# jenkinsm13/julia-spira

Hardware: AMD Instinct MI355X
Metric: Msamples/sec at 1920x1080 spp=64 depth=8; fraction of HBM roofline (higher is better)
Workload: dtype f64

## Files before the change

### julia-spira_amd/csrc/spira_device.h

```cpp
#pragma once
#include <hip/hip_runtime.h>
#include <stdint.h>
#include <type_traits>
#include "spira_fastdiv.h"
#include "spira_sky.h"

namespace spira {

__device__ __forceinline__ float sqrt_rn(float x) { return __builtin_sqrtf(x); }
__device__ __forceinline__ double sqrt_rn(double x) { return __builtin_sqrt(x); }

constexpr int kBlock = 256;
#ifndef SPIRA_WAVES_F32
#define SPIRA_WAVES_F32 5
#endif
#ifndef SPIRA_WAVES_F64
#define SPIRA_WAVES_F64 4
#endif
#define SPIRA_WAVES_PER_SIMD(T) (sizeof(T) == 8 ? SPIRA_WAVES_F64 : SPIRA_WAVES_F32)
constexpr uint32_t kMaxTries = 64;

template <class T> struct Vec { T x, y, z; };

template <class T> __device__ __forceinline__ Vec<T> mk(T x, T y, T z) { Vec<T> r; r.x = x; r.y = y; r.z = z; return r; }
// ... 830 lines not shown
        n = mk<T>(sc.tri[3 * ti].w, sc.tri[3 * ti + 1].w, sc.tri[3 * ti + 2].w);
    } else {
        const Pack4<T> e1p = sc.bvh_tris[3 * (size_t)slot + 1], e2p = sc.bvh_tris[3 * (size_t)slot + 2];
        n = normalize(cross(mk<T>(e1p.x, e1p.y, e1p.z), mk<T>(e2p.x, e2p.y, e2p.z)));
    }
    const int mi = material_of<T, BVH, TRI>(sc, prim, slot);
    const Pack4<T> ma = sc.mat[2 * mi], mb = sc.mat[2 * mi + 1];
    Vec<T> diffuse = mk<T>(ma.x, ma.y, ma.z), emission = mk<T>(mb.x, mb.y, mb.z);
    T specular = ma.w, roughness = mb.w;
    if (EXT && (ext->flags & kExtSpectral)) {
        const T sd = ext_uplift<T>(*ext, diffuse), se = ext_uplift<T>(*ext, emission);
        diffuse = mk<T>(sd, sd, sd); emission = mk<T>(se, se, se);
    }
    const bool has_contrib = (emission.x != 0 || emission.y != 0 || emission.z != 0);
    contrib = mulv(beta, emission);
    pend.kind = kDead; pend.rough = 0; pend.v = mk<T>(0, 0, 0);
    if (scatter) {
        if (EXT && (ext->flags & kExtDielectric) && roughness < (T)0.0) {
            pend.v = n; pend.kind = kDielectric; pend.rough = -roughness;
            beta = mulv(beta, diffuse);
        } else if (specular > (T)0.0) {
            pend.v = d - n * ((T)2 * dot(d, n));
            pend.kind = roughness > (T)0.0 ? kSpecRough : kMirror;
            pend.rough = roughness;
            beta = mulv(beta * specular, diffuse);
        } else {
            pend.v = pos + n;
            pend.kind = kDiffuse;
            beta = mulv(beta * (T)0.5, diffuse);
        }
    }
    return has_contrib;
}

template <class T, bool BVH, bool EXT = false>
__device__ __forceinline__ bool shade_hit(const SceneLds<T> &sc, const Vec<T> pos, const Vec<T> d, int prim, uint32_t slot, Vec<T> &beta,
                                          bool scatter, Vec<T> &contrib, Pending<T> &pend, const ExtState<T> *ext = nullptr) {
    ExactDiv exact;
    return shade_hit<T, BVH, EXT>(sc, pos, d, prim, slot, beta, scatter, contrib, pend, ext, exact);
}

template <class T>
__device__ __forceinline__ void dielectric_resolve(Pending<T> &pend, const Vec<T> d, const RngKey &key) {
    const Vec<T> n = pend.v;
    const T ior = pend.rough;
    const T cosd = dot(d, n);
    const bool entering = cosd < (T)0.0;
    const Vec<T> nn = entering ? n : mk<T>(-n.x, -n.y, -n.z);
    const T eta = entering ? (T)1.0 / ior : ior;
    const T ci = entering ? -cosd : cosd;
    const T s2 = (eta * eta) * ((T)1.0 - ci * ci);
    T r0 = ((T)1.0 - ior) / ((T)1.0 + ior); r0 = r0 * r0;
    const T x = (T)1.0 - ci, x2 = x * x;
    const T refl = r0 + ((T)1.0 - r0) * ((x2 * x2) * x);
    T u, u1, u2;
    rng3<T>(key, 1, u, u1, u2);
    if (s2 > (T)1.0 || u < refl) pend.v = d - nn * ((T)2 * dot(d, nn));
    else pend.v = d * eta + nn * (eta * ci - sqrt_rn((T)1.0 - s2));
    pend.kind = kMirror;
}

template <class T, bool BVH, bool EXT = false>
__device__ __forceinline__ SegInfo segment_front(const SceneLds<T> &sc, Vec<T> &o, const Vec<T> d, Vec<T> &beta, bool scatter,
                                                 Vec<T> &contrib, T &t_out, Pending<T> &pend, const ExtState<T> *ext = nullptr) {
    SegInfo info;
    T t;
    uint32_t slot;
    int prim = closest_hit<T, BVH>(sc, o, d, (T)0.001, t, slot);
    info.prim = prim;
    t_out = prim >= 0 ? t : (T)0;
    if (prim < 0) {
        pend.kind = kDead; pend.rough = 0; pend.v = mk<T>(0, 0, 0);
        contrib = sky_term_x<T, EXT>(d, beta, ext);
        info.alive = false; info.has_contrib = true;
        return info;
    }
    const Vec<T> pos = o + d * t;
    info.has_contrib = shade_hit<T, BVH, EXT>(sc, pos, d, prim, slot, beta, scatter, contrib, pend, ext);
    info.alive = scatter;
    if (scatter) o = pos;
    return info;
}

template <class T, class P>
__device__ __forceinline__ Vec<T> segment_back(const Vec<T> pos, const Pending<T> &pend, const Vec<T> rnd, P &pol) {
    if (pend.kind == kDiffuse) return normalize((pend.v + rnd) - pos, pol);
    Vec<T> reflected = pend.v;
    if (pend.kind == kSpecRough) reflected = reflected + rnd * pend.rough;
    return normalize(reflected, pol);
}
template <class T>
__device__ __forceinline__ Vec<T> segment_back(const Vec<T> pos, const Pending<T> &pend, const Vec<T> rnd) {
    ExactDiv exact;
    return segment_back<T>(pos, pend, rnd, exact);
}

template <class T, bool BVH, bool EXT = false>
__device__ __forceinline__ SegInfo trace_segment(const SceneLds<T> &sc, const RenderConst<T> &rc, Vec<T> &o, Vec<T> &d,
                                                 Vec<T> &beta, uint32_t pixel, uint32_t sample, uint32_t bounce,
                                                 bool scatter, Vec<T> &contrib, T &t_out, const ExtState<T> *ext = nullptr) {
    Pending<T> pend;
    const Vec<T> d_in = d;
    SegInfo info = segment_front<T, BVH, EXT>(sc, o, d, beta, scatter, contrib, t_out, pend, ext);
    if (info.alive) {
        Vec<T> rnd = mk<T>(0, 0, 0);
        if (EXT && pend.kind == kDielectric) dielectric_resolve<T>(pend, d_in, rng_key(rc.sA, rc.sB, pixel, sample, bounce));
        if (pend.kind == kDiffuse || pend.kind == kSpecRough)
            rnd = random_in_unit_sphere<T>(rng_key(rc.sA, rc.sB, pixel, sample, bounce));
        d = segment_back<T>(o, pend, rnd);
    }
    return info;
}

template <class T, class P>
__device__ __forceinline__ void camera_ray(const RenderConst<T> &rc, uint32_t i, uint32_t j, uint32_t pixel, uint32_t sample,
                                           Vec<T> &o, Vec<T> &d, P &pol) {
    T xu, xv, unused;
    rng3<T>(rng_key(rc.sA, rc.sB, pixel, sample, 0), 0, xu, xv, unused);
    T u = ((T)(i - 1) + xu) / (T)(rc.width - 1);
    T v = ((T)(j - 1) + xv) / (T)(rc.height - 1);
    o = rc.cam_origin;
    d = normalize(((rc.cam_llc + rc.cam_hor * u) + rc.cam_ver * v) - o, pol);
}
template <class T>
__device__ __forceinline__ void camera_ray(const RenderConst<T> &rc, uint32_t i, uint32_t j, uint32_t pixel, uint32_t sample,
                                           Vec<T> &o, Vec<T> &d) {
    ExactDiv exact;
    camera_ray<T>(rc, i, j, pixel, sample, o, d, exact);
}
__device__ __forceinline__ float to_scalar(float x) { return __uint_as_float(__builtin_amdgcn_readfirstlane(__float_as_uint(x))); }
__device__ __forceinline__ double to_scalar(double x) {
    const uint32_t lo = __builtin_amdgcn_readfirstlane((uint32_t)__double2loint(x)), hi = __builtin_amdgcn_readfirstlane((uint32_t)__double2hiint(x));
    return __hiloint2double((int)hi, (int)lo);
}
template <class T> struct PixelDiv { Recip<T> w1, h1; };
template <class T> __device__ __forceinline__ PixelDiv<T> pixel_divisors(const RenderConst<T> &rc) {
    PixelDiv<T> p;
    p.w1 = recip_of((T)(rc.width - 1)); p.h1 = recip_of((T)(rc.height - 1));
    p.w1.d = to_scalar(p.w1.d); p.w1.r = to_scalar(p.w1.r); p.h1.d = to_scalar(p.h1.d); p.h1.r = to_scalar(p.h1.r);
    return p;
}
template <class T> __device__ __forceinline__ T pixel_quotient(T n, const Recip<T> &rc, ExactDiv &) { return n / rc.d; }
template <class T> __device__ __forceinline__ T pixel_quotient(T n, const Recip<T> &rc, SpecDiv &) { return quotient(n, rc); }
template <class T, class P>
__device__ __forceinline__ void camera_ray_lds(const RenderConst<T> &rc, const T *cam, const PixelDiv<T> &pd, uint32_t i, uint32_t j, uint32_t pixel, uint32_t sample,
                                               Vec<T> &o, Vec<T> &d, P &pol) {
    T xu, xv, unused;
    rng3<T>(rng_key(rc.sA, rc.sB, pixel, sample, 0), 0, xu, xv, unused);
    T u = pixel_quotient<T>((T)(i - 1) + xu, pd.w1, pol);
    T v = pixel_quotient<T>((T)(j - 1) + xv, pd.h1, pol);
    o = mk<T>(cam[0], cam[1], cam[2]);
    const Vec<T> llc = mk<T>(cam[3], cam[4], cam[5]), hor = mk<T>(cam[6], cam[7], cam[8]), ver = mk<T>(cam[9], cam[10], cam[11]);
    d = normalize(((llc + hor * u) + ver * v) - o, pol);
}

template <class T>
__device__ __forceinline__ void path_of(const RenderConst<T> &rc, uint32_t q, uint32_t pass, uint32_t &i, uint32_t &j,
                                        uint32_t &pixel, uint32_t &sample) {
    uint32_t slot = fastdiv(q, rc.fd_tile);
    uint32_t pl = q - slot * rc.tile_pixels;
    uint32_t lr = fastdiv(pl, rc.fd_width);
    uint32_t lx = pl - lr * rc.width;
    j = ref_row_j(rc, lr);
    i = lx + 1;
    pixel = (j - 1) * rc.width + lx;
    sample = rc.sample0 + pass * rc.slots + slot;
}

template <class T> struct RayQueue { Pack4<T> *A; Pack4<T> *B; Pack2<T> *C; };

struct Stats {
    unsigned long long segments, rays_enqueued, radiance_rmw, radiance_store, redone_waves, rays_parked;
// ... 271 lines not shown
    uint32_t pass;
    uint32_t n_first;
    uint32_t dense_pct;
    Pack4<T> *mesh_list;
    uint32_t mesh_min_batch;
    uint32_t refill_free;
    uint32_t mesh_mode;
    uint32_t *mesh_count;
    uint32_t resume_k, resume_nw;
    uint32_t *redo;
    uint32_t redo_only;
    Stats *stats;
    Pack4<T> *accum;
    FastDiv fd_keff;
    uint32_t k_eff;
    uint32_t accum_first;
    uint32_t l_private;
    uint32_t sky_runs;
};

#ifndef SPIRA_RESOLVE_RUN
#define SPIRA_RESOLVE_RUN 4
#endif
__device__ __forceinline__ uint32_t owned_pixel(uint32_t w, uint32_t nw, uint32_t l) {
    constexpr uint32_t kRun = SPIRA_RESOLVE_RUN;
    static_assert(64 % kRun == 0, "a run length divides the wave");
    return ((l / kRun) * nw + w) * kRun + l % kRun;
}

template <class T>
__device__ __forceinline__ void resolve_pixel(Pack4<T> *accum, const Pack3<T> *L, uint32_t tile_pixels, uint32_t k_eff, bool first_pass, uint32_t p) {
    Pack4<T> acc;
    if (first_pass) { acc.x = 0; acc.y = 0; acc.z = 0; acc.w = 0; } else acc = accum[p];
    uint32_t s = 0;
    for (; s + 8 <= k_eff; s += 8) {
        Pack3<T> l[8];
#pragma unroll
        for (int k = 0; k < 8; ++k) l[k] = L[(size_t)(s + k) * tile_pixels + p];
#pragma unroll
        for (int k = 0; k < 8; ++k) { acc.x = acc.x + l[k].x; acc.y = acc.y + l[k].y; acc.z = acc.z + l[k].z; }
    }
    for (; s < k_eff; ++s) {
        const Pack3<T> l = L[(size_t)s * tile_pixels + p];
        acc.x = acc.x + l.x; acc.y = acc.y + l.y; acc.z = acc.z + l.z;
    }
    accum[p] = acc;
}
template <class T>
__device__ __forceinline__ void resolve_pixel_run(Pack4<T> *accum, const Pack3<T> *Lp, uint32_t k_eff, bool first_pass, uint32_t p) {
    constexpr uint32_t kRun = SPIRA_RESOLVE_RUN;
    Pack4<T> acc;
    if (first_pass) { acc.x = 0; acc.y = 0; acc.z = 0; acc.w = 0; } else acc = accum[p];
    uint32_t s = 0;
    for (; s + 8 <= k_eff; s += 8) {
        Pack3<T> l[8];
#pragma unroll
        for (int k = 0; k < 8; ++k) l[k] = Lp[(s + k) * kRun];
#pragma unroll
        for (int k = 0; k < 8; ++k) { acc.x = acc.x + l[k].x; acc.y = acc.y + l[k].y; acc.z = acc.z + l[k].z; }
    }
    for (; s < k_eff; ++s) {
        const Pack3<T> l = Lp[s * kRun];
        acc.x = acc.x + l.x; acc.y = acc.y + l.y; acc.z = acc.z + l.z;
    }
    accum[p] = acc;
}

__device__ __forceinline__ float pack_qref(uint32_t q, uint32_t, float) { return __uint_as_float(q); }
__device__ __forceinline__ double pack_qref(uint32_t q, uint32_t ref, double) { return __longlong_as_double((long long)((unsigned long long)q | ((unsigned long long)ref << 32))); }
__device__ __forceinline__ uint32_t unpack_q(float w) { return __float_as_uint(w); }
__device__ __forceinline__ uint32_t unpack_q(double w) { return (uint32_t)(unsigned long long)__double_as_longlong(w); }
__device__ __forceinline__ uint32_t unpack_ref(double w) { return (uint32_t)((unsigned long long)__double_as_longlong(w) >> 32); }

#ifdef SPIRA_MESH_STATS
__device__ unsigned long long g_mesh_dbg[32];
#define MESH_STAT(...) __VA_ARGS__
#else
#define MESH_STAT(...)
#endif

#ifndef SPIRA_CARRY_KEY
#define SPIRA_CARRY_KEY 1
#endif
#ifndef SPIRA_WAVES_B_F32
#define SPIRA_WAVES_B_F32 4
#endif
#ifndef SPIRA_WAVES_B_F64
#define SPIRA_WAVES_B_F64 SPIRA_WAVES_F64
#endif
#ifndef SPIRA_WAVES_PATH_F32
#define SPIRA_WAVES_PATH_F32 6
#endif
template <class T, int R, bool BVH, bool EXT, bool SPEC, int MODE = 0, bool TRI = true>
__global__ __launch_bounds__(kBlock, MODE == 2 ? (sizeof(T) == 8 ? SPIRA_WAVES_B_F64 : SPIRA_WAVES_B_F32) : (sizeof(T) == 4 ? SPIRA_WAVES_PATH_F32 : SPIRA_WAVES_F64)) void k_path(const PathArgs<T> a) {
    extern __shared__ __attribute__((aligned(32))) unsigned char lds_raw[];
    constexpr uint32_t WPB = kBlock / 64, SUB = 64 * R;
    constexpr bool kRefArray = sizeof(T) == 4;
    constexpr bool kCarry = SPIRA_CARRY_KEY && !BVH && !EXT;
    constexpr uint32_t kStageShift = 25, kRefMask = (1u << kStageShift) - 1u;
    const uint32_t lane = threadIdx.x & 63, wave = threadIdx.x >> 6;
    const uint32_t NW = gridDim.x * WPB, wid = blockIdx.x * WPB + wave;
    const RenderConst<T> &rc = a.rc;
    using Pol = typename std::conditional<SPEC, SpecDiv, ExactDiv>::type;
    Pol pol;
    if (!SPEC && a.redo_only) {
        uint32_t any = 0;
        for (uint32_t w = 0; w < WPB; ++w) any |= a.redo[blockIdx.x * WPB + w];
        if (!any) return;
    }
    T *cam_lds = reinterpret_cast<T *>(lds_raw + scene_lds_bytes<T>(a.scene.n_spheres, a.scene.n_materials, a.scene.n_triangles) + WPB * SUB * sizeof(Pack4<T>));
    if (threadIdx.x < 12) {
        const Vec<T> *cv = threadIdx.x < 3 ? &rc.cam_origin : (threadIdx.x < 6 ? &rc.cam_llc : (threadIdx.x < 9 ? &rc.cam_hor : &rc.cam_ver));
        const uint32_t cc = threadIdx.x % 3;
        cam_lds[threadIdx.x] = cc == 0 ? cv->x : (cc == 1 ? cv->y : cv->z);
    }
    Pack4<T> *cam_sph = reinterpret_cast<Pack4<T> *>(reinterpret_cast<unsigned char *>(cam_lds) + 128);
    constexpr bool kCam = !EXT;
    if (kCam && MODE != 2 && a.cam_consts)
        for (uint32_t i = threadIdx.x; i < a.scene.n_spheres; i += blockDim.x) {
            const T *sp = a.scene.spheres5 + 5 * (size_t)i;
            const Vec<T> oc = rc.cam_origin - mk<T>(sp[0], sp[1], sp[2]);
            Pack4<T> k; k.x = oc.x; k.y = oc.y; k.z = oc.z; k.w = dot(oc, oc) - sp[3] * sp[3];
            cam_sph[i] = k;
        }
    const SceneLds<T> sc = stage_scene<T>(a.scene, lds_raw);
    const PixelDiv<T> pix_div = pixel_divisors<T>(rc);
    if (!SPEC && a.redo_only) {
        if (!a.redo[wid]) return;
        if (lane == 0) atomicAdd(&a.stats->redone_waves, 1ull);
    }
    Pack4<T> *s_rnd = reinterpret_cast<Pack4<T> *>(lds_raw + scene_lds_bytes<T>(a.scene.n_spheres, a.scene.n_materials, a.scene.n_triangles)) + wave * SUB;
    constexpr uint32_t mesh_mode = BVH ? (uint32_t)MODE : 0u;
    const uint32_t kseg = mesh_mode == 2u ? a.resume_k : 1u;
    if (mesh_mode == 2u && wid * kseg >= a.resume_nw) return;
    const uint32_t region = wid * kseg * a.cap;
    const unsigned long long lt_mask = (1ull << lane) - 1ull;
    const uint32_t ref_base = sc.n_spheres + sc.n_triangles;
    const bool mixed = mesh_mode != 0u || rc.max_depth <= 128u;
    const uint32_t dense_pct = mixed ? a.dense_pct : 0u;
    const bool defer = mesh_mode != 0u || (BVH && mixed && a.mesh_list != nullptr);
    Pack4<T> *mlist = a.mesh_list + 3 * (size_t)region;
    uint32_t n_rmw = 0, n_store = 0, n_seg = 0, n_enq = 0, n_park = 0;
    uint32_t n_wtrips = 0, n_ltrips = 0;
    uint32_t n_in = 0;
    const bool own = !BVH && !EXT && !TRI && sizeof(T) == 8 && a.accum != nullptr;
    const uint32_t n_own = own ? 64u * a.k_eff : 0u;
    const uint32_t n_sub_first = own ? (n_own + SUB - 1) / SUB : (a.n_first + SUB - 1) / SUB;
    const bool priv = kCarry && own && a.l_private != 0;
    const uint32_t l_base = priv ? wid * n_own : 0u;
    constexpr bool kOwnT = !BVH && !EXT && !TRI && sizeof(T) == 8;
    uint32_t sky_mask = 0;
    uint32_t *sky_word = reinterpret_cast<uint32_t *>(cam_lds + 12) + wave;
    static_assert(12 * sizeof(T) + WPB * sizeof(uint32_t) <= 128 || !kOwnT, "a word per wave behind the camera");
    if constexpr (kOwnT) {
        if (own && a.sky_runs) {
            constexpr uint32_t kRun = SPIRA_RESOLVE_RUN, kRuns = 64 / kRun, kRowSlots = 64 / kRun;
            static_assert(kRun == 4 && 2 * 64 * sizeof(Pack3<T>) <= SUB * sizeof(Pack4<T>), "the run mask below is written for runs of 4; a row of terms fits the work list");
            {
                const uint32_t px = owned_pixel(wid, NW, lane);
                bool sky = false;
                if (px < rc.tile_pixels) {
                    uint32_t pi, pj, pixel, sample;
                    path_of<T>(rc, px, a.pass, pi, pj, pixel, sample);
                    sky = sky_pixel(cam_lds, rc.width, rc.height, pi, pj, a.scene.spheres5, a.scene.n_spheres);
                }
                unsigned long long b = __ballot(sky);
                b &= b >> 1; b &= b >> 2;
                for (uint32_t g = 0; g < kRuns; ++g) sky_mask |= (uint32_t)((b >> (kRun * g)) & 1ull) << g;
            }
            Pack3<T> *s_sky = reinterpret_cast<Pack3<T> *>(s_rnd);
            for (uint32_t m = sky_mask; m; m &= m - 1u) {
                const uint32_t g = (uint32_t)__builtin_ctz(m);
                const uint32_t px = owned_pixel(wid, NW, g * kRun + lane % kRun);
                uint32_t pi, pj, pixel, sample0;
                path_of<T>(rc, px, a.pass, pi, pj, pixel, sample0);
                Pack3<T> acc;
                acc.x = 0; acc.y = 0; acc.z = 0;
                if (!a.accum_first && lane < kRun) { const Pack4<T> a0 = a.accum[px]; acc.x = a0.x; acc.y = a0.y; acc.z = a0.z; }
                for (uint32_t s0 = 0; s0 < a.k_eff; s0 += kRowSlots) {
                    const uint32_t slot = s0 + lane / kRun;
                    if (slot < a.k_eff) {
                        Vec<T> o_, d_;
                        camera_ray_lds<T>(rc, cam_lds, pix_div, pi, pj, pixel, sample0 + slot, o_, d_, pol);
                        const Vec<T> c = sky_term_x<T, EXT>(d_, mk<T>(1, 1, 1), nullptr);
                        Pack3<T> l; l.x = c.x; l.y = c.y; l.z = c.z;
                        s_sky[lane] = l;
                        ++n_seg; ++n_store;
                    }
                    wave_lds_sync();
                    if (lane < kRun) {
                        const uint32_t n = a.k_eff - s0 < kRowSlots ? a.k_eff - s0 : kRowSlots;
                        for (uint32_t k = 0; k < n; ++k) { const Pack3<T> l = s_sky[k * kRun + lane]; acc.x = acc.x + l.x; acc.y = acc.y + l.y; acc.z = acc.z + l.z; }
                    }
                    wave_lds_sync();
                }
                if (lane < kRun) a.L[priv ? l_base + g * a.k_eff * kRun + lane : px] = acc;
            }
        }
        if (own) { if (lane == 0) *sky_word = sky_mask; wave_lds_sync(); }
    }

    auto park = [&](uint32_t slot_i, const Vec<T> o_, const Vec<T> d_, const Vec<T> beta_, T closest_, uint32_t q_, int prim_, uint32_t stage_hit) {
        Pack4<T> A, B, C;
        A.x = o_.x; A.y = o_.y; A.z = o_.z; A.w = d_.x;
        B.x = d_.y; B.y = d_.z; B.z = beta_.x; B.w = beta_.y;
        C.x = beta_.z; C.y = closest_; C.z = Bits<T>::from_u32(q_); C.w = Bits<T>::from_u32((uint32_t)(prim_ + 1) | (stage_hit << kStageShift));
        mlist[3 * (size_t)slot_i] = A; mlist[3 * (size_t)slot_i + 1] = B; mlist[3 * (size_t)slot_i + 2] = C;
    };
    uint32_t mfill = 0;
    constexpr int kMaxSeg = 16;
    uint32_t pfx[kMaxSeg + 1];
    bool segmented = false;
    {
        uint32_t cnt = 0;
        if (mesh_mode == 2u && lane < kseg && wid * kseg + lane < a.resume_nw) cnt = a.mesh_count[wid * kseg + lane];
        pfx[0] = 0;
#pragma unroll
        for (int j = 0; j < kMaxSeg; ++j) pfx[j + 1] = pfx[j] + (uint32_t)__builtin_amdgcn_readlane((int)cnt, j);
        if (mesh_mode == 2u) { mfill = pfx[kMaxSeg]; segmented = true; }
    }
    const uint32_t first_sub = own ? 0u : (mesh_mode == 1u ? (wid % a.resume_k) * (NW / a.resume_k) + wid / a.resume_k : wid);
    const uint32_t sub_step = own ? 1u : NW;
    MESH_STAT(unsigned long long dbg_t0 = __builtin_readcyclecounter(); unsigned long long dbg_sess = 0, dbg_walk = 0; uint32_t dbg_ns = 0, dbg_ws = 0, dbg_ls = 0, dbg_rf = 0, dbg_rays = 0, dbg_rounds = 0, dbg_ws1 = 0, dbg_ls1 = 0, dbg_h[4] = {0, 0, 0, 0};)
    for (uint32_t round = 0; ; ++round) {
        MESH_STAT(++dbg_rounds;)
        const bool first = mesh_mode != 2u && round == 0;
        const RayQueue<T> qin = a.q[(round + 1) & 1], qout = a.q[round & 1];
        const uint32_t *rin = a.qref[(round + 1) & 1];
        uint32_t *rout = a.qref[round & 1];
        const uint2 *kin = a.qkey[(round + 1) & 1];
        uint2 *kout = a.qkey[round & 1];
        const uint32_t limit = first ? (own ? n_own : a.n_first) : n_in;
        const uint32_t n_sub = first ? n_sub_first : (n_in + SUB - 1) / SUB;
        uint32_t fill = 0;
        for (uint32_t sub = first ? first_sub : 0u; sub < n_sub; sub += first ? sub_step : 1u) {
            if constexpr (kOwnT) if (own && first) {
                const uint32_t m = (uint32_t)__builtin_amdgcn_readfirstlane((int)*sky_word);
                const uint32_t r0 = fastdiv(sub * SUB / SPIRA_RESOLVE_RUN, a.fd_keff), r1 = fastdiv((sub * SUB + SUB - 1) / SPIRA_RESOLVE_RUN, a.fd_keff);
                if (r0 == r1 && ((m >> r0) & 1u)) continue;
            }
            Vec<T> o[R], beta[R];
            Pending<T> pend[R];
            ExtState<T> ex[R];
            uint32_t q[R], ent[R], stg[R], ref[R];
            uint32_t ka[R], kb[R];
            bool valid[R];
#pragma unroll
            for (int r = 0; r < R; ++r) {
                const uint32_t idx = sub * SUB + r * 64 + lane;
                valid[r] = false; stg[r] = round; ref[r] = 0; q[r] = 0; ka[r] = 0; kb[r] = 0;
                pend[r].kind = kDead; pend[r].rough = 0; pend[r].v = mk<T>(0, 0, 0);
                o[r] = mk<T>(0, 0, 0); beta[r] = mk<T>(1, 1, 1);
                bool parked = false; T park_t = 0; int park_prim = -1;
                uint32_t qf = idx;
                bool in = idx < limit;
                if (own && first) {
                    const uint32_t t = idx / SPIRA_RESOLVE_RUN, run = fastdiv(t, a.fd_keff);
                    const uint32_t px = owned_pixel(wid, NW, run * SPIRA_RESOLVE_RUN + idx % SPIRA_RESOLVE_RUN);
                    qf = (t - run * a.k_eff) * rc.tile_pixels + px;
                    in = in && px < rc.tile_pixels;
                    if constexpr (kOwnT) in = in && !((*sky_word >> run) & 1u);
                }
                const uint32_t ql = priv ? l_base + idx : qf;
                if (in) {
                    if (first) {
                        uint32_t pixel, sample, pi, pj;
                        Vec<T> d;
                        q[r] = ql;
                        path_of<T>(rc, qf, a.pass, pi, pj, pixel, sample);
                        if (kCarry) { ka[r] = mix32(rc.sA + pixel) ^ (sample << 8); kb[r] = mix32(rc.sB ^ pixel) + (sample << 8); }
                        camera_ray_lds<T>(rc, cam_lds, pix_div, pi, pj, pixel, sample, o[r], d, pol);
                        if (EXT) { ex[r].flags = rc.flags; if (rc.flags & kExtSpectral) beta[r] = ext_wavelength<T>(sc, rc.sA, rc.sB, pixel, sample, ex[r]); }
                        T t; uint32_t slot = 0;
                        int prim;
                        if (defer) {
                            if (kCam && a.cam_consts) closest_hit_local<T, Pol, TRI, true>(sc, o[r], d, (T)0.001, t, prim, pol, cam_sph);
                            else closest_hit_local<T, Pol, TRI>(sc, o[r], d, (T)0.001, t, prim, pol);
                            parked = mesh_box_hit<T>(sc, o[r], d, t);
                        } else if (kCam && !BVH && a.cam_consts) { closest_hit_local<T, Pol, TRI, true>(sc, o[r], d, (T)0.001, t, prim, pol, cam_sph); }
                        else prim = closest_hit<T, BVH, Pol, TRI>(sc, o[r], d, (T)0.001, t, slot, pol);
                        ++n_seg;
                        if (parked) { park_t = t; park_prim = prim; pend[r].v = d; }
                        else if (prim < 0) {
                            const Vec<T> c = sky_term_x<T, EXT>(d, beta[r], &ex[r]);
                            Pack3<T> l; l.x = c.x; l.y = c.y; l.z = c.z;
                            a.L[ql] = l;
                            ++n_store;
                        } else {
                            valid[r] = true;
                            o[r] = o[r] + d * t;
                            ref[r] = (BVH && prim >= (int)ref_base) ? ref_base + slot : (uint32_t)prim;
                            pend[r].v = d;
                        }
                    } else {
                        const Pack4<T> A = qin.A[region + idx], B = qin.B[region + idx];
                        const Pack2<T> C = qin.C[region + idx];
                        o[r] = mk<T>(A.x, A.y, A.z);
                        pend[r].v = mk<T>(A.w, B.x, B.y);
                        beta[r] = mk<T>(B.z, B.w, C.x);
                        q[r] = unpack_q(C.y);
                        uint32_t w;
                        if constexpr (kRefArray) w = rin[region + idx]; else w = unpack_ref(C.y);
                        if (mixed) { stg[r] = w >> kStageShift; ref[r] = w & kRefMask; } else ref[r] = w;
                        if (kCarry) { const uint2 k = kin[region + idx]; ka[r] = k.x; kb[r] = k.y; }
                        valid[r] = true;
                    }
                }
                if (defer && first) {
                    const unsigned long long mp = __ballot(parked);
                    if (parked) park(mfill + __popcll(mp & lt_mask), o[r], pend[r].v, beta[r], park_t, q[r], park_prim, 0u);
                    mfill += (uint32_t)__popcll(mp); n_park += (uint32_t)__popcll(mp);
                }
            }
            while (true) {
                uint32_t n_list = 0, n_valid = 0;
#pragma unroll
                for (int r = 0; r < R; ++r) {
                    bool want = false;
                    RngKey key;
                    const Vec<T> d = pend[r].v;
                    pend[r].kind = kDead;
                    if (valid[r]) {
                        uint32_t pixel = 0, sample = 0, pi, pj;
                        const bool scatter = stg[r] + 1 < rc.max_depth;
                        int prim = (int)ref[r]; uint32_t slot = 0;
                        if (BVH && ref[r] >= ref_base) { prim = (int)ref_base; slot = ref[r] - ref_base; }
                        const uint32_t qi = q[r] & 0x7FFFFFFFu;
                        const bool has_l = (q[r] >> 31) != 0;
                        if (EXT) {
                            path_of<T>(rc, qi, a.pass, pi, pj, pixel, sample);
                            ex[r].flags = rc.flags;
                            if (rc.flags & kExtSpectral) (void)ext_wavelength<T>(sc, rc.sA, rc.sB, pixel, sample, ex[r]);
                        }
                        Vec<T> contrib;
                        const bool has_contrib = shade_hit<T, BVH, EXT, Pol, TRI>(sc, o[r], d, prim, slot, beta[r], scatter, contrib, pend[r], &ex[r], pol);
                        if (has_contrib) {
                            Pack3<T> l; l.x = contrib.x; l.y = contrib.y; l.z = contrib.z;
                            if (has_l) { const Pack3<T> l0 = a.L[qi]; l.x = l0.x + contrib.x; l.y = l0.y + contrib.y; l.z = l0.z + contrib.z; ++n_rmw; }
                            else ++n_store;
                            a.L[qi] = l;
                            q[r] |= 0x80000000u;
                        } else if (!scatter && !has_l) {
                            Pack3<T> l; l.x = 0; l.y = 0; l.z = 0;
                            a.L[qi] = l;
                            ++n_store;
                        }
                        want = (pend[r].kind == kDiffuse || pend[r].kind == kSpecRough);
                        if (want || (EXT && pend[r].kind == kDielectric)) {
                            if (kCarry && mixed) {
                                key.hA = mix32(ka[r] ^ stg[r]); key.hB = mix32(kb[r] + stg[r]); key.hBr = (key.hB << 16) | (key.hB >> 16);
                            } else {
                                if (!EXT) path_of<T>(rc, qi, a.pass, pi, pj, pixel, sample);
                                key = rng_key(rc.sA, rc.sB, pixel, sample, stg[r]);
                            }
                            if (EXT && pend[r].kind == kDielectric) dielectric_resolve<T>(pend[r], d, key);
                        }
                    }
                    const unsigned long long mv = __ballot(pend[r].kind != kDead);
                    n_valid += (uint32_t)__popcll(mv);
                    const unsigned long long m = __ballot(want);
                    if (want) {
                        ent[r] = n_list + __popcll(m & lt_mask);
                        uint32_t *kw = reinterpret_cast<uint32_t *>(&s_rnd[ent[r]]);
                        kw[0] = key.hA; kw[1] = key.hB;
                    }
                    n_list += (uint32_t)__popcll(m);
                }
                if (n_valid == 0) break;
                wave_lds_sync();
                drain_unit_sphere_list<T>(s_rnd, n_list, lane);
                wave_lds_sync();
                uint32_t n_hit = 0;
#pragma unroll
                for (int r = 0; r < R; ++r) {
                    bool hit = false, parked3 = false;
                    T park_t3 = 0; int park_prim3 = -1;
                    if (pend[r].kind != kDead) {
                        Vec<T> rnd = mk<T>(0, 0, 0);
                        if (pend[r].kind != kMirror) rnd = RndTry<T>::load(&s_rnd[ent[r]]);
                        const Vec<T> nd = segment_back<T>(o[r], pend[r], rnd, pol);
                        T t; uint32_t slot = 0;
                        int prim;
                        if (defer) {
                            closest_hit_local<T, Pol, TRI>(sc, o[r], nd, (T)0.001, t, prim, pol);
                            parked3 = mesh_box_hit<T>(sc, o[r], nd, t);
                        } else prim = closest_hit<T, BVH, Pol, TRI>(sc, o[r], nd, (T)0.001, t, slot, pol);
                        ++n_seg;
                        if (parked3) { park_t3 = t; park_prim3 = prim; pend[r].v = nd; }
                        else if (prim < 0) {
                            const Vec<T> c = sky_term_x<T, EXT>(nd, beta[r], &ex[r]);
                            const uint32_t qi = q[r] & 0x7FFFFFFFu;
                            Pack3<T> l; l.x = c.x; l.y = c.y; l.z = c.z;
                            if (q[r] >> 31) { const Pack3<T> l0 = a.L[qi]; l.x = l0.x + c.x; l.y = l0.y + c.y; l.z = l0.z + c.z; ++n_rmw; }
                            else ++n_store;
                            a.L[qi] = l;
                        } else {
                            hit = true;
                            o[r] = o[r] + nd * t;
                            ref[r] = (BVH && prim >= (int)ref_base) ? ref_base + slot : (uint32_t)prim;
                            pend[r].v = nd;
                            ++stg[r];
                        }
                    }
                    if (defer) {
                        const unsigned long long mp = __ballot(parked3);
                        if (parked3) park(mfill + __popcll(mp & lt_mask), o[r], pend[r].v, beta[r], park_t3, q[r], park_prim3, stg[r] + 1u);
                        mfill += (uint32_t)__popcll(mp); n_park += (uint32_t)__popcll(mp);
                    }
                    valid[r] = hit;
                    n_hit += (uint32_t)__popcll(__ballot(hit));
                }
                wave_lds_sync();
                if (n_hit == 0) break;
                if (dense_pct && n_hit * 100u >= n_valid * dense_pct) continue;
#pragma unroll
                for (int r = 0; r < R; ++r) {
                    const unsigned long long m = __ballot(valid[r]);
                    if (valid[r]) {
                        const uint32_t dst = region + fill + __popcll(m & lt_mask);
                        const Vec<T> nd = pend[r].v;
                        const uint32_t w = mixed ? (ref[r] | (stg[r] << kStageShift)) : ref[r];
                        Pack4<T> A, B; Pack2<T> C;
                        A.x = o[r].x; A.y = o[r].y; A.z = o[r].z; A.w = nd.x;
                        B.x = nd.y; B.y = nd.z; B.z = beta[r].x; B.w = beta[r].y;
                        C.x = beta[r].z; C.y = pack_qref(q[r], w, (T)0);
                        qout.A[dst] = A; qout.B[dst] = B; qout.C[dst] = C;
                        if constexpr (kRefArray) rout[dst] = w;
                        if constexpr (kCarry) kout[dst] = make_uint2(ka[r], kb[r]);
                    }
                    fill += (uint32_t)__popcll(m);
                }
                break;
            }
        }
        if (defer && mesh_mode != 1u && mfill && (mfill >= a.mesh_min_batch || fill == 0)) {
            constexpr int kLdsStack = (int)(SUB * sizeof(Pack4<T>) / (64 * sizeof(uint32_t)));
            __builtin_amdgcn_fence(__ATOMIC_RELEASE, "workgroup");
            __builtin_amdgcn_fence(__ATOMIC_ACQUIRE, "workgroup");
            uint32_t *lstack = reinterpret_cast<uint32_t *>(s_rnd);
            uint32_t stack[kBvhStackD - kLdsStack];
            uint32_t next = 0;
            MESH_STAT(const unsigned long long dbg_s0 = __builtin_readcyclecounter(); ++dbg_ns; dbg_rays += mfill;)
#ifdef SPIRA_BVH_SCREEN
            constexpr bool kScreened = sizeof(T) == 8;
#else
            constexpr bool kScreened = false;
#endif
            if constexpr (kScreened) {
            bool walking = false, finished = false, full = false;
            uint32_t ent_i = 0;
            float dxf = 0, dyf = 0, dzf = 1;
            Bvh8Ray ry; ry.ox = ry.oy = ry.oz = 0; ry.ix = ry.iy = ry.iz = 1; ry.oct = 0; ry.best = 0; ry.tmin = 0; ry.amin = 0;
            Bvh8Walk<T> wk; wk.G = 0; wk.tw = 0; wk.rank = 0; wk.sp = 0; wk.t0 = 0; wk.c0 = wk.c1 = wk.c2 = wk.c3 = 0; wk.nc = 0;
            auto decode = [&](const Pack4<T> A, const Pack4<T> B, const Pack4<T> C, Vec<T> &o_, Vec<T> &d_, Vec<T> &beta_, T &closest, uint32_t &q_, int &prim, uint32_t &slot, uint32_t &stage_hit) {
                o_ = mk<T>(A.x, A.y, A.z); d_ = mk<T>(A.w, B.x, B.y); beta_ = mk<T>(B.z, B.w, C.x);
                closest = C.y;
                q_ = Bits<T>::to_u32(C.z);
                const uint32_t pw = Bits<T>::to_u32(C.w);
                prim = (int)(pw & kRefMask) - 1;
                stage_hit = pw >> kStageShift;
                slot = 0;
                if (prim >= (int)ref_base) { slot = (uint32_t)prim - ref_base; prim = (int)ref_base; }
            };
// ... 127 lines not shown
                        const Vec<T> hp = o_ + d_ * closest;
                        const uint32_t w_ = ((prim >= (int)ref_base) ? ref_base + slot : (uint32_t)prim) | (stage_hit << kStageShift);
                        const uint32_t dst = region + fill + __popcll(mh & lt_mask);
                        Pack4<T> A, B; Pack2<T> C;
                        A.x = hp.x; A.y = hp.y; A.z = hp.z; A.w = d_.x;
                        B.x = d_.y; B.y = d_.z; B.z = beta_.x; B.w = beta_.y;
                        C.x = beta_.z; C.y = pack_qref(q_, w_, (T)0);
                        qout.A[dst] = A; qout.B[dst] = B; qout.C[dst] = C;
                        if constexpr (kRefArray) rout[dst] = w_;
                    }
                }
                fill += (uint32_t)__popcll(mh);
                finished = false;
                const unsigned long long mf = __ballot(!walking);
                const uint32_t take = min((uint32_t)__popcll(mf), mfill - next);
                if (!walking && (uint32_t)__popcll(mf & lt_mask) < take) {
                    const uint32_t e = next + (uint32_t)__popcll(mf & lt_mask);
                    const Pack4<T> *ent = mlist + 3 * (size_t)e;
                    if (segmented) {
                        uint32_t seg = 0, off = e;
#pragma unroll
                        for (int j = 1; j < kMaxSeg; ++j) if (e >= pfx[j]) { seg = (uint32_t)j; off = e - pfx[j]; }
                        ent = a.mesh_list + 3 * ((size_t)(wid * kseg + seg) * a.cap + off);
                    }
                    const Pack4<T> A = ent[0], B = ent[1], C = ent[2];
                    o_ = mk<T>(A.x, A.y, A.z); d_ = mk<T>(A.w, B.x, B.y); beta_ = mk<T>(B.z, B.w, C.x);
                    closest = C.y;
                    q_ = Bits<T>::to_u32(C.z);
                    const uint32_t pw = Bits<T>::to_u32(C.w);
                    prim = (int)(pw & kRefMask) - 1;
                    stage_hit = pw >> kStageShift;
                    slot = 0;
                    T t0;
                    if (bvh8_enter<T>(sc, o_, d_, closest, ry, t0)) { bvh8_begin<T>(wk, ry, t0, (T)0.001, sc.bvh_root[2].w); walking = true; }
                    else finished = true;
                }
                next += take;
                if (!__any(walking)) { if (__any(finished)) continue; break; }
                const bool more = next < mfill;
                MESH_STAT(++dbg_rf; const unsigned long long dbg_w0 = __builtin_readcyclecounter();)
                uint32_t n_now = (uint32_t)__popcll(__ballot(walking));
                while (true) {
                    ++n_wtrips; n_ltrips += n_now;
                    MESH_STAT(++dbg_ws; { const uint32_t nl = (uint32_t)__popcll(__ballot(walking)); dbg_ls += nl; if (segmented) { ++dbg_ws1; dbg_ls1 += nl; } ++dbg_h[nl <= 8 ? 0 : (nl <= 24 ? 1 : (nl <= 48 ? 2 : 3))]; })
                    if (walking && !bvh8_step<T, kLdsStack>(sc, wk, ry, o_, d_, (T)0.001, (int)ref_base, closest, prim, slot, lstack, stack, lane)) { walking = false; finished = true; }
                    const uint32_t n_walk = (uint32_t)__popcll(__ballot(walking));
                    n_now = n_walk;
                    if (n_walk == 0 || (more && 64u - n_walk >= a.refill_free)) break;
                }

                MESH_STAT(dbg_walk += __builtin_readcyclecounter() - dbg_w0;)
            }
            }
            mfill = 0;
            segmented = false;
            MESH_STAT(dbg_sess += __builtin_readcyclecounter() - dbg_s0;)
        }
        n_in = fill;
        n_enq += fill;
        if (n_in == 0 && (mfill == 0 || mesh_mode == 1u)) break;
        __builtin_amdgcn_fence(__ATOMIC_RELEASE, "workgroup");
        __builtin_amdgcn_fence(__ATOMIC_ACQUIRE, "workgroup");
    }
    for (int sft = 32; sft > 0; sft >>= 1) { n_rmw += __shfl_down(n_rmw, sft); n_seg += __shfl_down(n_seg, sft); n_store += __shfl_down(n_store, sft); }
    const bool again = SPEC && __any(outside_window<T>(pol));
    if (own && !again && !(SPEC && a.redo_only == 2u)) {
        __builtin_amdgcn_fence(__ATOMIC_RELEASE, "workgroup");
        __builtin_amdgcn_fence(__ATOMIC_ACQUIRE, "workgroup");
        const uint32_t px = owned_pixel(wid, NW, lane);
        bool summed = false;
        if constexpr (kOwnT) sky_mask = (uint32_t)__builtin_amdgcn_readfirstlane((int)*sky_word);
        if constexpr (kOwnT) summed = ((sky_mask >> (lane / SPIRA_RESOLVE_RUN)) & 1u) != 0;
        if (summed) {
            const Pack3<T> l = a.L[priv ? l_base + (lane / SPIRA_RESOLVE_RUN) * a.k_eff * SPIRA_RESOLVE_RUN + lane % SPIRA_RESOLVE_RUN : px];
            Pack4<T> acc;
            if (a.accum_first) acc.w = 0; else acc = a.accum[px];
            acc.x = l.x; acc.y = l.y; acc.z = l.z;
            a.accum[px] = acc;
        } else if (px < rc.tile_pixels) {
            if (priv) resolve_pixel_run<T>(a.accum, a.L + l_base + (lane / SPIRA_RESOLVE_RUN) * a.k_eff * SPIRA_RESOLVE_RUN + lane % SPIRA_RESOLVE_RUN, a.k_eff, a.accum_first != 0, px);
            else resolve_pixel<T>(a.accum, a.L, rc.tile_pixels, a.k_eff, a.accum_first != 0, px);
        }
        const uint32_t seg = __shfl(n_seg, 0), rmw = __shfl(n_rmw, 0), sto = __shfl(n_store, 0);
        if (lane < 4) {
            unsigned long long *f = lane == 0 ? &a.stats->segments : (lane == 1 ? &a.stats->rays_enqueued : (lane == 2 ? &a.stats->radiance_rmw : &a.stats->radiance_store));
            atomicAdd(f, (unsigned long long)(lane == 0 ? seg : (lane == 1 ? n_enq : (lane == 2 ? rmw : sto))));
        }
        if constexpr (kOwnT) if (lane == 4 && sky_mask) atomicAdd(&a.stats->sky_pixels, (unsigned long long)(SPIRA_RESOLVE_RUN * __popc(sky_mask)));
    }
    MESH_STAT(if (lane == 0) { unsigned long long *g = g_mesh_dbg + (mesh_mode == 2u ? 16 : 0);
                               atomicAdd(&g[0], __builtin_readcyclecounter() - dbg_t0); atomicAdd(&g[1], dbg_sess); atomicAdd(&g[2], (unsigned long long)dbg_ns);
                               atomicAdd(&g[3], (unsigned long long)dbg_ws); atomicAdd(&g[4], (unsigned long long)dbg_ls); atomicAdd(&g[5], (unsigned long long)dbg_rf);
                               atomicAdd(&g[6], (unsigned long long)dbg_rays); atomicAdd(&g[7], (unsigned long long)dbg_rounds); atomicAdd(&g[9], dbg_walk); atomicAdd(&g[10], 1ull); atomicAdd(&g[11], (unsigned long long)dbg_ws1); atomicAdd(&g[12], (unsigned long long)dbg_ls1);
                               atomicAdd(&g[8], (unsigned long long)dbg_h[0]); atomicAdd(&g[13], (unsigned long long)dbg_h[1]); atomicAdd(&g[14], (unsigned long long)dbg_h[2]); atomicAdd(&g[15], (unsigned long long)dbg_h[3]); })
    if (lane == 0) {
        if (mesh_mode == 2u) {
            const uint32_t row = 4 * wid * kseg;
            a.blk_stats[row] += n_seg; a.blk_stats[row + 1] += n_rmw; a.blk_stats[row + 2] += n_store; a.blk_stats[row + 3] += n_enq;
        } else {
            a.blk_stats[4 * wid] = n_seg;
            a.blk_stats[4 * wid + 1] = n_rmw;
            a.blk_stats[4 * wid + 2] = n_store;
            a.blk_stats[4 * wid + 3] = n_enq;
            if (mesh_mode == 1u) a.mesh_count[wid] = mfill;
        }
        if (SPEC) a.redo[wid] = again ? 1u : 0u;
        if (BVH && n_park && !again && !(SPEC && a.redo_only == 2u)) atomicAdd(&a.stats->rays_parked, (unsigned long long)n_park);
        if (BVH && mesh_mode != 1u && n_wtrips && !again && !(SPEC && a.redo_only == 2u)) { atomicAdd(&a.stats->mesh_wave_trips, (unsigned long long)n_wtrips); atomicAdd(&a.stats->mesh_lane_trips, (unsigned long long)n_ltrips); }
    }
}

template <class T, bool BVH, bool EXT>
__global__ __launch_bounds__(kBlock) void k_mega(const BounceArgs<T> a) {
    extern __shared__ __attribute__((aligned(32))) unsigned char lds_raw[];
    const SceneLds<T> sc = stage_scene<T>(a.scene, lds_raw);
    const RenderConst<T> &rc = a.rc;
    unsigned long long nseg = 0;
    const uint32_t stride = gridDim.x * kBlock;
    uint32_t idx = blockIdx.x * kBlock + threadIdx.x;
    bool fresh = true;
    uint32_t pixel = 0, sample = 0, b = 0;
    Vec<T> o = mk<T>(0, 0, 0), d = mk<T>(0, 0, 1), beta = mk<T>(1, 1, 1), Lacc = mk<T>(0, 0, 0);
    ExtState<T> ex; ex.flags = rc.flags; ex.bR = 0; ex.bG = 0; ex.bB = 0;
    while (idx < a.n_first) {
        if (fresh) {
            uint32_t pi, pj;
            path_of<T>(rc, idx, a.pass, pi, pj, pixel, sample);
            camera_ray<T>(rc, pi, pj, pixel, sample, o, d);
            beta = mk<T>(1, 1, 1); Lacc = mk<T>(0, 0, 0); b = 0;
            if (EXT && (rc.flags & kExtSpectral)) beta = ext_wavelength<T>(sc, rc.sA, rc.sB, pixel, sample, ex);
            fresh = false;
        }
        Vec<T> contrib; T t_hit;
        SegInfo si = trace_segment<T, BVH, EXT>(sc, rc, o, d, beta, pixel, sample, b, b + 1 < rc.max_depth, contrib, t_hit, &ex);
        ++nseg;
        if (b == 0) { if (si.has_contrib) Lacc = contrib; }
        else if (si.has_contrib) Lacc = Lacc + contrib;
        ++b;
        if (!si.alive || b == rc.max_depth) {
            Pack3<T> l; l.x = Lacc.x; l.y = Lacc.y; l.z = Lacc.z;
            a.L[idx] = l;
            idx += stride;
            fresh = true;
        }
    }
    for (int sft = 32; sft > 0; sft >>= 1) nseg += __shfl_down(nseg, sft);
    if ((threadIdx.x & 63) == 0 && nseg) atomicAdd(&a.stats->segments, nseg);
}

template <class T, bool BVH, bool EXT>
__global__ __launch_bounds__(64) void k_trace(const BounceArgs<T> a, const uint32_t *ijs, uint32_t n_paths, int *prims, T *ts,
                                              T *dirs, T *radiance) {
    extern __shared__ __attribute__((aligned(32))) unsigned char lds_raw[];
    const SceneLds<T> sc = stage_scene<T>(a.scene, lds_raw);
    const RenderConst<T> &rc = a.rc;
    uint32_t p = blockIdx.x * blockDim.x + threadIdx.x;
    if (p >= n_paths) return;
    uint32_t i = ijs[3 * p], j = ijs[3 * p + 1], sample = ijs[3 * p + 2];
    uint32_t pixel = (j - 1) * rc.width + (i - 1);
    Vec<T> o, d, beta = mk<T>(1, 1, 1), Lacc = mk<T>(0, 0, 0);
    camera_ray<T>(rc, i, j, pixel, sample, o, d);
    ExtState<T> ex; ex.flags = rc.flags; ex.bR = 0; ex.bG = 0; ex.bB = 0;
    if (EXT && (rc.flags & kExtSpectral)) beta = ext_wavelength<T>(sc, rc.sA, rc.sB, pixel, sample, ex);
    for (uint32_t b = 0; b < rc.max_depth; ++b) {
        Vec<T> contrib; T t_hit;
        Vec<T> dir_in = d;
        SegInfo si = trace_segment<T, BVH, EXT>(sc, rc, o, d, beta, pixel, sample, b, b + 1 < rc.max_depth, contrib, t_hit, &ex);
        size_t k = (size_t)p * rc.max_depth + b;
        prims[k] = si.prim; ts[k] = t_hit;
        dirs[3 * k] = dir_in.x; dirs[3 * k + 1] = dir_in.y; dirs[3 * k + 2] = dir_in.z;
        if (b == 0) { if (si.has_contrib) Lacc = contrib; }
// ... 756 lines not shown
```

Before: 27810.

## Merge normalize paths, spread sky accumulation across lanes, reorder key loads, fuse stat atomics

```diff
diff --git a/julia-spira_amd/csrc/spira_device.h b/julia-spira_amd/csrc/spira_device.h
--- a/julia-spira_amd/csrc/spira_device.h
+++ b/julia-spira_amd/csrc/spira_device.h
@@ -936,12 +936,22 @@
     return info;
 }
 
-template <class T, class P>
+#ifndef SPIRA_ONE_NORMALIZE
+#define SPIRA_ONE_NORMALIZE 1
+#endif
+template <class T, class P, bool ONE = (SPIRA_ONE_NORMALIZE != 0)>
 __device__ __forceinline__ Vec<T> segment_back(const Vec<T> pos, const Pending<T> &pend, const Vec<T> rnd, P &pol) {
-    if (pend.kind == kDiffuse) return normalize((pend.v + rnd) - pos, pol);
-    Vec<T> reflected = pend.v;
-    if (pend.kind == kSpecRough) reflected = reflected + rnd * pend.rough;
-    return normalize(reflected, pol);
+    if constexpr (ONE) {
+        Vec<T> v = pend.v;
+        if (pend.kind == kDiffuse) v = (pend.v + rnd) - pos;
+        else if (pend.kind == kSpecRough) v = pend.v + rnd * pend.rough;
+        return normalize(v, pol);
+    } else {
+        if (pend.kind == kDiffuse) return normalize((pend.v + rnd) - pos, pol);
+        Vec<T> reflected = pend.v;
+        if (pend.kind == kSpecRough) reflected = reflected + rnd * pend.rough;
+        return normalize(reflected, pol);
+    }
 }
 template <class T>
 __device__ __forceinline__ Vec<T> segment_back(const Vec<T> pos, const Pending<T> &pend, const Vec<T> rnd) {
@@ -1379,6 +1389,12 @@
 #ifndef SPIRA_CARRY_KEY
 #define SPIRA_CARRY_KEY 1
 #endif
+#ifndef SPIRA_KEYS_CONSUMED
+#define SPIRA_KEYS_CONSUMED 1
+#endif
+#ifndef SPIRA_SKY_LANES12
+#define SPIRA_SKY_LANES12 1
+#endif
 #ifndef SPIRA_WAVES_B_F32
 #define SPIRA_WAVES_B_F32 4
 #endif
@@ -1394,6 +1410,7 @@
     constexpr uint32_t WPB = kBlock / 64, SUB = 64 * R;
     constexpr bool kRefArray = sizeof(T) == 4;
     constexpr bool kCarry = SPIRA_CARRY_KEY && !BVH && !EXT;
+    constexpr bool kOneNorm = SPIRA_ONE_NORMALIZE && sizeof(T) == 8 && !BVH;
     constexpr uint32_t kStageShift = 25, kRefMask = (1u << kStageShift) - 1u;
     const uint32_t lane = threadIdx.x & 63, wave = threadIdx.x >> 6;
     const uint32_t NW = gridDim.x * WPB, wid = blockIdx.x * WPB + wave;
@@ -1471,9 +1488,16 @@
                 const uint32_t px = owned_pixel(wid, NW, g * kRun + lane % kRun);
                 uint32_t pi, pj, pixel, sample0;
                 path_of<T>(rc, px, a.pass, pi, pj, pixel, sample0);
+#if SPIRA_SKY_LANES12
+                const uint32_t px_c = owned_pixel(wid, NW, g * kRun + (lane < 3 * kRun ? lane / 3 : 0u));
+                const T *s_val = reinterpret_cast<const T *>(s_sky);
+                T acc_c = 0;
+                if (!a.accum_first && lane < 3 * kRun) acc_c = reinterpret_cast<const T *>(a.accum + px_c)[lane % 3];
+#else
                 Pack3<T> acc;
                 acc.x = 0; acc.y = 0; acc.z = 0;
                 if (!a.accum_first && lane < kRun) { const Pack4<T> a0 = a.accum[px]; acc.x = a0.x; acc.y = a0.y; acc.z = a0.z; }
+#endif
                 for (uint32_t s0 = 0; s0 < a.k_eff; s0 += kRowSlots) {
                     const uint32_t slot = s0 + lane / kRun;
                     if (slot < a.k_eff) {
@@ -1485,13 +1509,24 @@
                         ++n_seg; ++n_store;
                     }
                     wave_lds_sync();
+#if SPIRA_SKY_LANES12
+                    if (lane < 3 * kRun) {
+                        const uint32_t n = a.k_eff - s0 < kRowSlots ? a.k_eff - s0 : kRowSlots;
+                        for (uint32_t k = 0; k < n; ++k) acc_c = acc_c + s_val[3 * kRun * k + lane];
+                    }
+#else
                     if (lane < kRun) {
                         const uint32_t n = a.k_eff - s0 < kRowSlots ? a.k_eff - s0 : kRowSlots;
                         for (uint32_t k = 0; k < n; ++k) { const Pack3<T> l = s_sky[k * kRun + lane]; acc.x = acc.x + l.x; acc.y = acc.y + l.y; acc.z = acc.z + l.z; }
                     }
+#endif
                     wave_lds_sync();
                 }
+#if SPIRA_SKY_LANES12
+                if (lane < 3 * kRun) reinterpret_cast<T *>(a.L + (priv ? l_base + g * a.k_eff * kRun + lane / 3 : px_c))[lane % 3] = acc_c;
+#else
                 if (lane < kRun) a.L[priv ? l_base + g * a.k_eff * kRun + lane : px] = acc;
+#endif
             }
         }
         if (own) { if (lane == 0) *sky_word = sky_mask; wave_lds_sync(); }
@@ -1590,6 +1625,9 @@
                             pend[r].v = d;
                         }
                     } else {
+#if SPIRA_KEYS_CONSUMED
+                        if (kCarry) { const uint2 k = kin[region + idx]; ka[r] = k.x; kb[r] = k.y; }
+#endif
                         const Pack4<T> A = qin.A[region + idx], B = qin.B[region + idx];
                         const Pack2<T> C = qin.C[region + idx];
                         o[r] = mk<T>(A.x, A.y, A.z);
@@ -1599,7 +1637,9 @@
                         uint32_t w;
                         if constexpr (kRefArray) w = rin[region + idx]; else w = unpack_ref(C.y);
                         if (mixed) { stg[r] = w >> kStageShift; ref[r] = w & kRefMask; } else ref[r] = w;
+#if !SPIRA_KEYS_CONSUMED
                         if (kCarry) { const uint2 k = kin[region + idx]; ka[r] = k.x; kb[r] = k.y; }
+#endif
                         valid[r] = true;
                     }
                 }
@@ -1675,7 +1715,7 @@
                     if (pend[r].kind != kDead) {
                         Vec<T> rnd = mk<T>(0, 0, 0);
                         if (pend[r].kind != kMirror) rnd = RndTry<T>::load(&s_rnd[ent[r]]);
-                        const Vec<T> nd = segment_back<T>(o[r], pend[r], rnd, pol);
+                        const Vec<T> nd = segment_back<T, Pol, kOneNorm>(o[r], pend[r], rnd, pol);
                         T t; uint32_t slot = 0;
                         int prim;
                         if (defer) {
@@ -1969,11 +2009,18 @@
             else resolve_pixel<T>(a.accum, a.L, rc.tile_pixels, a.k_eff, a.accum_first != 0, px);
         }
         const uint32_t seg = __shfl(n_seg, 0), rmw = __shfl(n_rmw, 0), sto = __shfl(n_store, 0);
+#if SPIRA_SKY_LANES12
+        if (lane < 4 || (kOwnT && lane == 4 && sky_mask)) {
+            unsigned long long *f = lane == 0 ? &a.stats->segments : (lane == 1 ? &a.stats->rays_enqueued : (lane == 2 ? &a.stats->radiance_rmw : (lane == 3 ? &a.stats->radiance_store : &a.stats->sky_pixels)));
+            atomicAdd(f, (unsigned long long)(lane == 0 ? seg : (lane == 1 ? n_enq : (lane == 2 ? rmw : (lane == 3 ? sto : SPIRA_RESOLVE_RUN * (uint32_t)__popc(sky_mask))))));
+        }
+#else
         if (lane < 4) {
             unsigned long long *f = lane == 0 ? &a.stats->segments : (lane == 1 ? &a.stats->rays_enqueued : (lane == 2 ? &a.stats->radiance_rmw : &a.stats->radiance_store));
             atomicAdd(f, (unsigned long long)(lane == 0 ? seg : (lane == 1 ? n_enq : (lane == 2 ? rmw : sto))));
         }
         if constexpr (kOwnT) if (lane == 4 && sky_mask) atomicAdd(&a.stats->sky_pixels, (unsigned long long)(SPIRA_RESOLVE_RUN * __popc(sky_mask)));
+#endif
     }
     MESH_STAT(if (lane == 0) { unsigned long long *g = g_mesh_dbg + (mesh_mode == 2u ? 16 : 0);
                                atomicAdd(&g[0], __builtin_readcyclecounter() - dbg_t0); atomicAdd(&g[1], dbg_sess); atomicAdd(&g[2], (unsigned long long)dbg_ns);
```

Result: no change. 28210 (median of 6 runs) (+1.5%).
